# pabloconrat/our_first_climate_model

Hardware: NVIDIA B200
Metric: column*wavelength*layer flux updates/s (repwvl-100 RCE step) (higher is better)
Workload: dtype f64

## Files before the change

our_first_climate_model_b200/csrc/rcm_capi.cu:

```cuda
#include <algorithm>
#include <cmath>
#include <cstdio>
#include <cstdlib>
#include <cstring>
#include <new>
#include <functional>
#include <string>
#include <vector>

#include "rcm_diag.cuh"

#ifndef M_PI
#define M_PI 3.14159265358979323846
#endif

struct rcm_solver {
    int device = 0;
    cudaStream_t own_stream = nullptr, stream = nullptr;
    rcm_params p{};
    DevConst dc{};
    bool const_dirty = true;
    int opt_angle_cubes = 1;
    int opt_angle_pairs = 1;
    int opt_config = 0;
// ... 27 lines not shown
    bool lbl_mode = false;
    int lbl_nwvl = 0;
    double lbl_co2_factor = 1.0;
    bool lbl_has_o3_ref = false;
    double *d_lbl_lo = nullptr, *d_lbl_hi = nullptr, *d_lbl_tau5 = nullptr, *d_lbl_h2o_ref = nullptr,
           *d_lbl_o3_ref = nullptr, *d_sH = nullptr, *d_sO = nullptr, *d_dTstat = nullptr, *d_part = nullptr;
    size_t part_cap = 0;
    unsigned char* d_tile = nullptr;
    double* d_spart = nullptr;
    unsigned* d_counter = nullptr;
    unsigned* d_multi = nullptr;
    size_t multi_cap = 0;
    int opt_multi = 1;
    size_t tile_cap = 0, spart_cap = 0;
    bool tile_vmr_valid = false;
    std::vector<double> stage;
    std::string err;
    long launches = 0;
    std::vector<std::pair<cudaEvent_t, cudaEvent_t>> ev_free, ev_used;
    cudaStream_t pipe_stream[3] = {nullptr, nullptr, nullptr};
    cudaEvent_t pipe_done[3] = {nullptr, nullptr, nullptr}, pipe_start = nullptr;
    struct HostGraph {
        cudaGraphExec_t exec = nullptr;
        SplitArgs sig{};
        const void* host[7] = {};
        const void* dev[4] = {};
        double dT_converged = 0.0;
        int ncol = 0, nchunk = 0, nkernels = 0;
        long captures = 0, replays = 0;
        bool failed = false;
// ... 240 lines not shown
    CU(dalloc(s->d_rh, n * NLAY));
    CU(dalloc(s->d_Tprev, n * NLAY));
    CU(dalloc(s->d_time, n));
    CU(dalloc(s->d_Ed, n * NLEV));
    CU(dalloc(s->d_Eu, n * NLEV));
    CU(dalloc(s->d_dE, n * NLAY));
    CU(dalloc(s->d_dt, n));
    CU(dalloc(s->d_lowpos, n * NLAY));
    s->cap = ncol;
    s->diag_steps = 0;
    s->part_cap = 0;
    s->tile_cap = s->spart_cap = 0;
    s->tile_vmr_valid = false;
    if (s->d_dTstat) cudaFree(s->d_dTstat);
    s->d_dTstat = nullptr;
    if (s->d_solar_col) cudaFree(s->d_solar_col);
    if (s->d_cloud_col) cudaFree(s->d_cloud_col);
    s->d_solar_col = s->d_cloud_col = nullptr;
    s->has_col_solar = s->has_col_cloud = false;
    return RCM_OK;
}

int ensure_diag(rcm_solver* s, int nsteps) {
    if ((size_t)nsteps <= s->diag_steps && s->d_diag) return RCM_OK;
    CU(dalloc(s->d_diag, (size_t)nsteps * s->cap * 4));
    CU(dalloc(s->d_scalars, (size_t)nsteps * 4));
    CU(dalloc(s->d_red, rcm_reduce_scratch_doubles(nsteps)));
    CU(dalloc(s->d_ticket, (size_t)nsteps));
    CU(cudaMemsetAsync(s->d_ticket, 0, (size_t)nsteps * sizeof(unsigned), s->stream));
    s->diag_steps = nsteps;
// ... 90 lines not shown


bool use_split(const rcm_solver* s) {
    return !s->lbl_mode && s->has_table && s->nactive == 5 && s->opt_config == 0 && s->opt_path == 0;
}

struct SplitGeom { int ntiles, nitem, nsplit; };
SplitGeom split_geom(const rcm_solver* s, int ncols) {
    SplitGeom g;
    g.ntiles = (ncols + 15) / 16;
    g.nitem = (s->dc.nwvl + 3) / 4;
    g.nsplit = (g.nitem + rcm_split_ipu() - 1) / rcm_split_ipu();
    return g;
}

int ensure_split(rcm_solver* s) {
    const SplitGeom g = split_geom(s, s->cap);
    const size_t tiles = (size_t)g.ntiles, need_part = tiles * g.nsplit * rcm_split_part_doubles();
    if (tiles > s->tile_cap || !s->d_tile) {
        CU(dalloc(s->d_tile, tiles * rcm_split_tile_bytes()));
        s->tile_cap = tiles;
        s->tile_vmr_valid = false;
    }
    if (need_part > s->spart_cap || !s->d_spart) {
        CU(dalloc(s->d_spart, need_part));
        s->spart_cap = need_part;
    }
    if (tiles > s->multi_cap || !s->d_multi) {
        if (s->d_multi) CU(cudaFree(s->d_multi));
        s->d_multi = nullptr;
        CU(cudaMalloc((void**)&s->d_multi, 2 * tiles * sizeof(unsigned)));
        s->multi_cap = tiles;
    }
    if (!s->d_dTstat) CU(dalloc(s->d_dTstat, (size_t)s->cap));
    if (!s->d_counter) {
        CU(dalloc(s->d_counter, (size_t)4));
        CU(cudaMemsetAsync(s->d_counter, 0, 4 * sizeof(unsigned), s->stream));
    }
    return RCM_OK;
}

SplitArgs split_args(rcm_solver* s, int col0, int ncols, int which) {
    const SplitGeom g = split_geom(s, ncols);
    const size_t o = (size_t)col0, t0 = o / 16;
    SplitArgs a{};
    a.ncol = ncols;
    a.diag_ncol = s->ncol;
    a.ntiles = g.ntiles;
    a.nsplit = g.nsplit;
// ... 15 lines not shown
    a.rel_hum = s->d_rh + o * NLAY;
    a.Tprev = s->d_Tprev + o * NLAY;
    a.time_h = s->d_time + o;
    a.E_down = s->d_Ed + o * NLEV;
    a.E_up = s->d_Eu + o * NLEV;
    a.dE = s->d_dE + o * NLAY;
    a.dt = s->d_dt + o;
    a.diag = s->d_diag + o * 4;
    a.solar_col = s->has_col_solar ? s->d_solar_col + o : nullptr;
    a.cloud_col = s->has_col_cloud ? s->d_cloud_col + o : nullptr;
    a.tile = s->d_tile + t0 * rcm_split_tile_bytes();
    a.part = s->d_spart + t0 * g.nsplit * rcm_split_part_doubles();
    a.dTstat = s->d_dTstat + o;
    a.counter = s->d_counter + which;
    a.quota = 1 << 30;
    return a;
}

int split_grid(const rcm_solver* s, const SplitArgs& a, int nsm) {
    (void)s;
    if (a.quota < a.nunits) return (a.nunits + a.quota - 1) / a.quota;
    int per_sm = 3;
    if (const char* e = std::getenv("RCM_CTAS_PER_SM")) {
        const int v = std::atoi(e);
        if (v >= 1 && v < per_sm) per_sm = v;
    }
    return std::min(a.nunits, nsm * per_sm);
}

int split_rt(rcm_solver* s, const SplitArgs& a, int nsm, cudaStream_t st, bool timed) {
// ... 10 lines not shown
    }
    CU(rcm_launch_split_rt(a, split_grid(s, a, nsm), st));
    s->launches += 1;
    if (timed) {
        CU(cudaEventRecord(ev.second, st));
        s->ev_used.push_back(ev);
        if (s->ev_used.size() >= 1024) {
            const int rc = rcm_kernel_time_ms(s, 0, nullptr, nullptr);
            if (rc != RCM_OK) return rc;
        }
    }
    return RCM_OK;
}

int split_advance(rcm_solver* s, int nsteps) {
    int st = refresh_const(s);
    if (st != RCM_OK) return st;
    st = ensure_split(s);
    if (st != RCM_OK) return st;
    const int nsm = nsm_of(s);
    const SplitArgs a = split_args(s, 0, s->ncol, 0);
    SplitColFlags f{};
    f.prep = 1;
    f.first = (s->step_index == 0);
    f.write_all_vmr = !s->tile_vmr_valid;
    CU(rcm_launch_split_col(a, f, s->stream));
    s->launches += 1;
    s->tile_vmr_valid = true;
    static const int multi_rounds = std::getenv("RCM_MULTI_ROUNDS") ? std::atoi(std::getenv("RCM_MULTI_ROUNDS")) : 24;
    const int grid1 = split_grid(s, a, nsm);
    const bool few_rounds = a.nunits < (long long)multi_rounds * grid1;
    const bool fits = (long long)a.nunits * nsteps + 2LL * grid1 < (1LL << 31);
    if (nsteps >= 2 && fits && (s->opt_multi == 2 || (s->opt_multi == 1 && few_rounds))) {
        SplitMultiArgs m{};
        m.nsteps = nsteps;
        m.done = s->d_multi;
        m.ready = s->d_multi + a.ntiles;
        CU(cudaMemsetAsync(s->d_multi, 0, 2 * (size_t)a.ntiles * sizeof(unsigned), s->stream));
        SplitArgs am = a;
        am.quota = 1 << 30;
        CU(rcm_launch_split_multi(am, m, split_grid(s, am, nsm), s->stream));
        s->launches += 1;
        return RCM_OK;
    }
    for (int k = 0; k < nsteps; ++k) {
        st = split_rt(s, a, nsm, s->stream, k < 4);
        if (st != RCM_OK) return st;
        SplitColFlags e{};
        e.finish = 1;
        e.prep = (k + 1 < nsteps);
        e.first = 0;
        e.write_out = (k + 1 == nsteps);
        e.diag_step = k;
        CU(rcm_launch_split_col(a, e, s->stream));
        s->launches += 1;
    }
    return RCM_OK;
}

int launch(rcm_solver* s, int mode, int nsteps, bool want_diag) {
    int st = refresh_const(s);
    if (st != RCM_OK) return st;
    if (mode == MODE_RT ? !s->has_spectral : !s->has_table) return fail(s, RCM_ERR_STATE, "no lookup table loaded");
    if (s->ncol <= 0) return fail(s, RCM_ERR_STATE, "no columns loaded");
    const int nsm = nsm_of(s);
    Part parts[2];
    const int nparts = plan_parts(s, s->ncol, nsm, parts);
    std::pair<cudaEvent_t, cudaEvent_t> ev;
    if (!s->ev_free.empty()) {
        ev = s->ev_free.back();
        s->ev_free.pop_back();
// ... 210 lines not shown
        return RCM_ERR_CUDA;
    }
    set_active_species(s);
    *out = s;
    return RCM_OK;
}

int rcm_destroy(rcm_solver* s) {
    if (!s) return RCM_OK;
    cudaSetDevice(s->device);
    cudaStreamSynchronize(s->stream);
    if (g_const_owner[s->device & 63] == s) g_const_owner[s->device & 63] = nullptr;
    void* ptrs[] = {s->d_coef3, s->d_xsec_file, s->d_coef, s->d_species, s->d_planck_c, s->d_planck_k, s->d_exp_tab, s->d_T, s->d_Ts, s->d_vmr, s->d_rh,
                    s->d_Tprev, s->d_time, s->d_lbl_lo, s->d_lbl_hi, s->d_lbl_tau5, s->d_lbl_h2o_ref, s->d_lbl_o3_ref, s->d_sH, s->d_sO,
                    s->d_dTstat, s->d_part, s->d_Ed, s->d_Eu, s->d_dE, s->d_dt, s->d_diag, s->d_scalars, s->d_red, s->d_tau,
                    s->d_lowpos, s->d_solar_col, s->d_cloud_col, s->d_ticket, s->d_tile, s->d_spart, s->d_counter, s->d_multi, s->d_diagnose};
    for (void* q : ptrs)
        if (q) cudaFree(q);
    for (auto& e : s->ev_free) { cudaEventDestroy(e.first); cudaEventDestroy(e.second); }
    for (auto& e : s->ev_used) { cudaEventDestroy(e.first); cudaEventDestroy(e.second); }
    for (int i = 0; i < 3; ++i) {
        if (s->pipe_stream[i]) cudaStreamDestroy(s->pipe_stream[i]);
        if (s->pipe_done[i]) cudaEventDestroy(s->pipe_done[i]);
    }
    if (s->pipe_start) cudaEventDestroy(s->pipe_start);
    for (cudaStream_t q : {s->sp_up, s->sp_rt[0], s->sp_rt[1], s->sp_down})
        if (q) cudaStreamDestroy(q);
    for (int i = 0; i < 24; ++i) {
        if (s->sp_prep[i]) cudaEventDestroy(s->sp_prep[i]);
        if (s->sp_rtdone[i]) cudaEventDestroy(s->sp_rtdone[i]);
    }
// ... 1 lines not shown
    for (int i = 0; i < 2; ++i) {
        if (s->dg_stream[i]) cudaStreamDestroy(s->dg_stream[i]);
        if (s->dg_join[i]) cudaEventDestroy(s->dg_join[i]);
    }
    if (s->dg_fork) cudaEventDestroy(s->dg_fork);
    if (s->hg.exec) cudaGraphExecDestroy(s->hg.exec);
    if (s->own_stream) cudaStreamDestroy(s->own_stream);
    delete s;
    return RCM_OK;
}

const char* rcm_last_error(const rcm_solver* s) { return s ? s->err.c_str() : "null solver"; }

int rcm_set_params(rcm_solver* s, const rcm_params* p) {
    if (!s || !p) return RCM_ERR_ARG;
    if (p->nangle < 1 || p->nangle > MAX_ANGLE || p->cloud_layer >= RCM_NLAYER) return fail(s, RCM_ERR_ARG, "bad params");
    unsigned old = s->p.species_mask;
    s->p = *p;
    if (old != p->species_mask) {
        s->coef_dirty = true;
        s->ncol = 0;
    }
    s->const_dirty = true;
    set_active_species(s);
    return RCM_OK;
}

int rcm_set_option(rcm_solver* s, int option, int value) {
    if (!s) return RCM_ERR_ARG;
    if (option == 0) {
        s->opt_angle_cubes = value ? 1 : 0;
        s->const_dirty = true;
        return RCM_OK;
    }
    if (option == 1) {
        s->opt_config = value;
        s->tile_vmr_valid = false;
        return RCM_OK;
    }
    if (option == 2) {
        s->opt_cplk_narrow = value ? 1 : 0;
        return RCM_OK;
    }
    if (option == 3) {
// ... 7 lines not shown
    }
    if (option == 5) {
        s->opt_path = value ? 1 : 0;
        s->tile_vmr_valid = false;
        return RCM_OK;
    }
    if (option == 6) {
        s->opt_multi = value < 0 ? 0 : value > 2 ? 2 : value;
        return RCM_OK;
    }
    return fail(s, RCM_ERR_ARG, "unknown option");
}

int rcm_set_stream(rcm_solver* s, void* cuda_stream) {
    if (!s) return RCM_ERR_ARG;
    s->stream = cuda_stream ? (cudaStream_t)cuda_stream : s->own_stream;
    return RCM_OK;
}

int rcm_synchronize(rcm_solver* s) {
    if (!s) return RCM_ERR_ARG;
    CU(cudaSetDevice(s->device));
    CU(cudaStreamSynchronize(s->stream));
    return RCM_OK;
}

int rcm_set_repwvl_table(rcm_solver* s, const double* xsec, const double* wvl, const double* weight,
                         const double* p_grid, const double* t_ref, const double* t_pert, int n_tpert, int n_species,
                         int n_wvl, int n_p) {
    if (!s || !xsec || !wvl || !weight || !p_grid || !t_ref || !t_pert) return RCM_ERR_ARG;
    if (n_tpert < 2 || n_tpert > MAX_TPERT || n_species != RCM_NSPECIES || n_wvl < 1 || n_p < 2)
        return fail(s, RCM_ERR_ARG, "unsupported table dimensions");
    CU(cudaSetDevice(s->device));
    const size_t n = (size_t)n_tpert * n_species * n_wvl * n_p;
    CU(dalloc(s->d_xsec_file, n));
    CU(cudaMemcpy(s->d_xsec_file, xsec, n * sizeof(double), cudaMemcpyHostToDevice));
    s->coef_dirty = true;
    {
        int st = rcm_set_spectral_grid(s, wvl, weight, n_wvl);
        if (st != RCM_OK) return st;
    }
    s->p_grid.assign(p_grid, p_grid + n_p);
    s->t_ref.assign(t_ref, t_ref + n_p);
    s->t_pert.assign(t_pert, t_pert + n_tpert);
    s->dc.nwvl = n_wvl;
    s->dc.n_tpert = n_tpert;
    s->dc.n_species = n_species;
    s->dc.n_p = n_p;
    for (int m = 0; m < n_tpert; ++m) s->dc.t_pert[m] = t_pert[m];
    s->has_table = true;
    s->lbl_mode = false;
    s->const_dirty = true;
    s->tau_valid = false;
    s->tau_cap = 0;
    return RCM_OK;
}

int rcm_set_spectral_grid(rcm_solver* s, const double* wvl, const double* weight, int n_wvl) {
    if (!s || !wvl || !weight || n_wvl < 1) return RCM_ERR_ARG;
    CU(cudaSetDevice(s->device));
    const double h = 6.62607e-34, c = 299792458, kB = 1.380649e-23;
    std::vector<double> pc(n_wvl), pk(n_wvl);
    double pc_max = 0.0;
    for (int i = 0; i < n_wvl; ++i) {
        const double lam = wvl[i] * 1e-9;
        pc[i] = h * c / (lam * kB);
        pk[i] = weight[i] * 2 * h * std::pow(c, 2) / std::pow(lam, 5) / 1e9;
        if (!(wvl[i] > 0.0) || !std::isfinite(pk[i])) return fail(s, RCM_ERR_ARG, "wavelengths must be positive and finite");
        pc_max = std::max(pc_max, pc[i]);
    }
    if (pc_max / 690.0 > 20.0)
        return fail(s, RCM_ERR_ARG, "wavelengths below 1043 nm are not supported (thermal solver: the Planck exponent would leave the range of the kernels' exp)");
    s->T_floor = pc_max / 690.0;
    CU(dalloc(s->d_planck_c, (size_t)n_wvl));
// ... 11 lines not shown
    s->lbl_mode = false;
    s->const_dirty = true;
    s->tau_valid = false;
    return RCM_OK;
}

int rcm_set_repwvl_table_from(rcm_solver* s, const rcm_table* t) {
    if (!s || !t) return RCM_ERR_ARG;
    return rcm_set_repwvl_table(s, t->xsec.data(), t->wvl.data(), t->weight.data(), t->p_grid.data(), t->t_ref.data(),
                                t->t_pert.data(), t->n_tpert, t->n_species, t->n_wvl, t->n_p);
}

int rcm_set_lbl_tables(rcm_solver* s, const double* wvl, const double* tau5, int nwvl, const double* h2o_ref,
                       const double* o3_ref, double co2_factor) {
    if (!s || !wvl || !tau5 || nwvl < 2 || !h2o_ref) return RCM_ERR_ARG;
    for (int i = 1; i < nwvl; ++i)
        if (!(wvl[i] > wvl[i - 1])) return fail(s, RCM_ERR_ARG, "LBL wavelengths must be strictly ascending");
    CU(cudaSetDevice(s->device));
    std::vector<double> lo(nwvl), hi(nwvl);
    for (int i = 0; i < nwvl; ++i) {
        const double dl = (i > 0) ? (wvl[i] - wvl[i - 1]) : (wvl[1] - wvl[0]);
        const double dh = (i < nwvl - 1) ? (wvl[i + 1] - wvl[i]) : (wvl[i] - wvl[i - 1]);
        lo[i] = wvl[i] - dl / 2.0;
        hi[i] = wvl[i] + dh / 2.0;
    }
    const size_t n = (size_t)nwvl;
    CU(dalloc(s->d_lbl_lo, 4 * n));
    CU(dalloc(s->d_lbl_hi, n));
    CU(dalloc(s->d_lbl_tau5, 3 * n * NLAY));
    CU(dalloc(s->d_lbl_h2o_ref, (size_t)NLAY));
// ... 28 lines not shown
    s->lbl_mode = true;
    if (s->dc.nwvl != nwvl) {
        s->has_table = s->has_spectral = false;
        s->tau_cap = 0;
    }
    s->tau_valid = false;
    s->dc.nwvl = nwvl;
    s->const_dirty = true;
    s->part_cap = 0;
    return RCM_OK;
}

int rcm_set_columns(rcm_solver* s, int ncol, const double* plevel_hPa, const double* Tlayer, const double* Tsurf,
                    const double* vmr9, const double* rel_hum) {
    if (!s || ncol <= 0 || !plevel_hPa || !Tlayer || !Tsurf || !vmr9 || !rel_hum) return RCM_ERR_ARG;
    CU(cudaSetDevice(s->device));
    int st = ensure_columns(s, ncol);
    if (st != RCM_OK) return st;
    s->ncol = ncol;
    if (!s->has_plevel || std::memcmp(s->plevel, plevel_hPa, sizeof(s->plevel)) != 0) s->coef_dirty = true;
    std::memcpy(s->plevel, plevel_hPa, sizeof(s->plevel));
    s->has_plevel = true;
    s->const_dirty = true;
    set_active_species(s);
    const size_t n = (size_t)ncol;
    s->stage.resize(n * s->nactive * NLAY);
    for (size_t c = 0; c < n; ++c)
        for (int k = 0; k < s->nactive; ++k)
            std::memcpy(&s->stage[(c * s->nactive + k) * NLAY], vmr9 + (c * RCM_NSPECIES + s->species[k]) * NLAY,
                        NLAY * sizeof(double));
// ... 2 lines not shown
    CU(cudaMemcpyAsync(s->d_Tprev, Tlayer, n * NLAY * sizeof(double), cudaMemcpyHostToDevice, s->stream));
    CU(cudaMemcpyAsync(s->d_Ts, Tsurf, n * sizeof(double), cudaMemcpyHostToDevice, s->stream));
    CU(cudaMemcpyAsync(s->d_rh, rel_hum, n * NLAY * sizeof(double), cudaMemcpyHostToDevice, s->stream));
    CU(cudaMemsetAsync(s->d_time, 0, n * sizeof(float), s->stream));
    CU(cudaStreamSynchronize(s->stream));
    s->step_index = 0;
    s->tau_valid = false;
    s->tile_vmr_valid = false;
    s->has_col_solar = s->has_col_cloud = false;
    return RCM_OK;
}

int rcm_set_column_solar(rcm_solver* s, const rcm_solar_params* sp, const double* tau_s, const double* mu_s,
                         const double* albedo, int cloud_from_tau_s, double* solar_irr_out, double* r_total_out) {
    if (!s) return RCM_ERR_ARG;
    if (s->ncol <= 0) return fail(s, RCM_ERR_STATE, "rcm_set_columns first");
    CU(cudaSetDevice(s->device));
    if (!sp) {
        s->has_col_solar = s->has_col_cloud = false;
        s->tau_valid = false;
        return RCM_OK;
    }
    if (sp->doublings < 0 || sp->doublings > 60) return fail(s, RCM_ERR_ARG, "doublings must be in 0..60");
    if (cloud_from_tau_s && s->p.cloud_layer < 0) return fail(s, RCM_ERR_ARG, "cloud_from_tau_s needs a cloud layer");
    const size_t n = (size_t)s->ncol;
    if (!s->d_solar_col) {
        CU(dalloc(s->d_solar_col, (size_t)s->cap));
        CU(dalloc(s->d_cloud_col, (size_t)s->cap));
    }
    double* d_in = nullptr;
// ... 25 lines not shown
    if (e == cudaSuccess && r_total_out)
        e = cudaMemcpyAsync(r_total_out, d_rt, n * sizeof(double), cudaMemcpyDeviceToHost, s->stream);
    if (e == cudaSuccess) e = cudaStreamSynchronize(s->stream);
    cudaFree(d_in);
    if (d_rt) cudaFree(d_rt);
    if (e != cudaSuccess) return cuda_fail(s, e, "rcm_set_column_solar");
    s->launches += 1;
    s->has_col_solar = true;
    s->has_col_cloud = cloud_from_tau_s != 0;
    s->tau_valid = false;
    return RCM_OK;
}

int rcm_update_columns(rcm_solver* s, const double* Tlayer, const double* Tsurf, const double* vmr_active) {
    if (!s) return RCM_ERR_ARG;
    if (s->ncol <= 0) return fail(s, RCM_ERR_STATE, "rcm_set_columns first");
    CU(cudaSetDevice(s->device));
    const size_t n = (size_t)s->ncol;
    if (Tlayer) CU(cudaMemcpyAsync(s->d_T, Tlayer, n * NLAY * sizeof(double), cudaMemcpyHostToDevice, s->stream));
    if (Tsurf) CU(cudaMemcpyAsync(s->d_Ts, Tsurf, n * sizeof(double), cudaMemcpyHostToDevice, s->stream));
    if (vmr_active)
        CU(cudaMemcpyAsync(s->d_vmr, vmr_active, n * s->nactive * NLAY * sizeof(double), cudaMemcpyHostToDevice, s->stream));
    if (vmr_active) s->tile_vmr_valid = false;
    s->tau_valid = false;
    return RCM_OK;
}

int rcm_set_step_index(rcm_solver* s, long step_index) {
    if (!s || step_index < 0) return RCM_ERR_ARG;
    s->step_index = step_index;
    return RCM_OK;
}

int rcm_build_tau(rcm_solver* s, double* tau_out, int* lowpos_p, int* lowpos_t) {
    if (!s) return RCM_ERR_ARG;
    if (s->lbl_mode) return fail(s, RCM_ERR_STATE, "rcm_build_tau is the repwvl read_tau: set a repwvl table after rcm_set_lbl_tables");
    if (!s->has_table || s->ncol <= 0) return fail(s, RCM_ERR_STATE, "table and columns must be loaded");
    CU(cudaSetDevice(s->device));
    int st = ensure_tau(s);
    if (st != RCM_OK) return st;
    st = launch(s, MODE_TAU, 1, false);
    if (st != RCM_OK) return st;
    const size_t n = (size_t)s->ncol;
    if (tau_out)
        CU(cudaMemcpyAsync(tau_out, s->d_tau, n * s->dc.nwvl * NLAY * sizeof(double), cudaMemcpyDeviceToHost, s->stream));
    std::vector<int> lt;
    if (lowpos_t) CU(cudaMemcpyAsync(lowpos_t, s->d_lowpos, n * NLAY * sizeof(int), cudaMemcpyDeviceToHost, s->stream));
    CU(cudaStreamSynchronize(s->stream));
    if (lowpos_p)
        for (size_t c = 0; c < n; ++c)
            for (int k = 0; k < NLAY; ++k) lowpos_p[c * NLAY + k] = s->dc.ip[NLAY - 1 - k];
    s->tau_valid = true;
    return RCM_OK;
}

int rcm_radiative_transfer(rcm_solver* s, const double* tau, double* E_down, double* E_up, double* dE) {
    if (!s) return RCM_ERR_ARG;
    if (s->lbl_mode) return fail(s, RCM_ERR_STATE, "rcm_radiative_transfer needs a repwvl spectral grid: set one after rcm_set_lbl_tables");
    if (!s->has_spectral || s->ncol <= 0) return fail(s, RCM_ERR_STATE, "spectral grid and columns must be loaded");
    CU(cudaSetDevice(s->device));
    int st = ensure_tau(s);
    if (st != RCM_OK) return st;
    const size_t n = (size_t)s->ncol;
    if (tau) {
        CU(cudaMemcpyAsync(s->d_tau, tau, n * s->dc.nwvl * NLAY * sizeof(double), cudaMemcpyHostToDevice, s->stream));
    } else if (!s->tau_valid) {
        return fail(s, RCM_ERR_STATE, "no tau: pass one or call rcm_build_tau first");
    }
    st = launch(s, MODE_RT, 1, false);
    if (st != RCM_OK) return st;
    if (E_down) CU(cudaMemcpyAsync(E_down, s->d_Ed, n * NLEV * sizeof(double), cudaMemcpyDeviceToHost, s->stream));
    if (E_up) CU(cudaMemcpyAsync(E_up, s->d_Eu, n * NLEV * sizeof(double), cudaMemcpyDeviceToHost, s->stream));
// ... 93 lines not shown
}

int rcm_advance(rcm_solver* s, int nsteps, rcm_step_scalars* scalars_out) {
    int st = rcm_advance_async(s, nsteps, nullptr);
    if (st != RCM_OK) return st;
    if (scalars_out) {
        CU(cudaMemcpyAsync(scalars_out, s->d_scalars, (size_t)nsteps * sizeof(rcm_step_scalars), cudaMemcpyDeviceToHost,
                           s->stream));
        CU(cudaStreamSynchronize(s->stream));
    }
    return RCM_OK;
}

int rcm_run_to_equilibrium(rcm_solver* s, long max_steps, int check_every, rcm_step_scalars* last, long* steps_done) {
    if (!s || max_steps <= 0 || check_every <= 0) return RCM_ERR_ARG;
    if (steps_done) *steps_done = 0;
    std::vector<rcm_step_scalars> sc((size_t)check_every);
    long done = 0;
    while (done < max_steps) {
        const int n = (int)std::min<long>(check_every, max_steps - done);
        const int st = rcm_advance(s, n, sc.data());
        if (st != RCM_OK) return st;
        done += n;
        if (last) *last = sc[n - 1];
        if (steps_done) *steps_done = done;
        if (sc[n - 1].n_converged >= (double)s->ncol) break;
    }
    return RCM_OK;
}

// ... 11 lines not shown
    if (dE) CU(cudaMemcpyAsync(dE, s->d_dE, n * NLAY * sizeof(double), cudaMemcpyDeviceToHost, s->stream));
    if (dt) CU(cudaMemcpyAsync(dt, s->d_dt, n * sizeof(double), cudaMemcpyDeviceToHost, s->stream));
    if (h2o) {
        if (s->h2o_slot < 0) return fail(s, RCM_ERR_STATE, "H2O is not an active species");
        CU(cudaMemcpy2DAsync(h2o, NLAY * sizeof(double), s->d_vmr + (size_t)s->h2o_slot * NLAY,
                             (size_t)s->nactive * NLAY * sizeof(double), NLAY * sizeof(double), n, cudaMemcpyDeviceToHost,
                             s->stream));
    }
    CU(cudaStreamSynchronize(s->stream));
    return RCM_OK;
}

int rcm_diagnose_fluxes(rcm_solver* s, int col0, int ncol, const double* vmr_scale, double* E_down_spec, double* E_up_spec,
                        double* E_down, double* E_up, double* dE) {
    if (!s) return RCM_ERR_ARG;
    if (s->lbl_mode) return fail(s, RCM_ERR_STATE, "rcm_diagnose_fluxes: the line-by-line path is not supported");
    if (!s->has_table) return fail(s, RCM_ERR_STATE, "rcm_diagnose_fluxes: no lookup table loaded");
    if (s->ncol <= 0) return fail(s, RCM_ERR_STATE, "rcm_diagnose_fluxes: no columns loaded");
    if (s->nactive != 5) return fail(s, RCM_ERR_STATE, "rcm_diagnose_fluxes: needs the five active species of the default species_mask");
    if (!use_split(s)) return fail(s, RCM_ERR_STATE, "rcm_diagnose_fluxes: needs the split path (RCM_OPT_PATH 0, no forced tile shape)");
    if (col0 < 0 || ncol <= 0 || (long long)col0 + ncol > s->ncol)
        return fail(s, RCM_ERR_ARG, "rcm_diagnose_fluxes: columns [" + std::to_string(col0) + ", " + std::to_string((long long)col0 + ncol) +
                                        ") outside the " + std::to_string(s->ncol) + " loaded");
    DiagScale sc{};
    for (int k = 0; k < 5; ++k) {
        sc.f[k] = vmr_scale ? vmr_scale[k] : 1.0;
        if (!(sc.f[k] >= 0.0) || !std::isfinite(sc.f[k]))
            return fail(s, RCM_ERR_ARG, "rcm_diagnose_fluxes: vmr_scale[" + std::to_string(k) + "] must be finite and >= 0");
    }
    CU(cudaSetDevice(s->device));
// ... 140 lines not shown
    for (int k = 0; k < na && ok; ++k) {
        buf.resize(arr[k].bytes);
        cudaError_t e = cudaMemcpy(buf.data(), arr[k].dev, arr[k].bytes, cudaMemcpyDeviceToHost);
        if (e != cudaSuccess) {
            std::fclose(f);
            return cuda_fail(s, e, "checkpoint download");
        }
        ok = std::fwrite(buf.data(), 1, arr[k].bytes, f) == arr[k].bytes;
    }
    ok = (std::fclose(f) == 0) && ok;
    return ok ? RCM_OK : fail(s, RCM_ERR_IO, std::string("short write to ") + path);
}

int rcm_load_checkpoint(rcm_solver* s, const char* path) {
    if (!s || !path) return RCM_ERR_ARG;
    CU(cudaSetDevice(s->device));
    CU(cudaStreamSynchronize(s->stream));
    FILE* f = std::fopen(path, "rb");
    if (!f) return fail(s, RCM_ERR_IO, std::string("cannot read ") + path);
    char magic[8];
    long long hdr[8];
    double plevel[RCM_NLEVEL];
    if (std::fread(magic, 1, 8, f) != 8 || std::memcmp(magic, "RCMCKPT1", 8) != 0 || std::fread(hdr, sizeof(hdr), 1, f) != 1 ||
        std::fread(plevel, sizeof(plevel), 1, f) != 1 || hdr[0] <= 0 || hdr[0] > (1LL << 30)) {
        std::fclose(f);
        return fail(s, RCM_ERR_FORMAT, std::string(path) + " is not a checkpoint of this solver");
    }
    set_active_species(s);
    if ((unsigned)hdr[2] != s->p.species_mask || (int)hdr[1] != s->nactive) {
        std::fclose(f);
// ... 43 lines not shown
    if (!s->has_plevel || std::memcmp(s->plevel, plevel, sizeof(plevel)) != 0) s->coef_dirty = true;
    std::memcpy(s->plevel, plevel, sizeof(plevel));
    s->has_plevel = true;
    s->const_dirty = true;
    s->step_index = (long)hdr[3];
    s->has_col_solar = hdr[4] != 0;
    s->has_col_cloud = hdr[5] != 0;
    s->tau_valid = false;
    s->tile_vmr_valid = false;
    return RCM_OK;
}

int rcm_step_host(rcm_solver* s, const double* Tlayer_in, const double* Tsurf_in, const double* vmr_active_in,
                  double* E_down, double* E_up, double* dE, double* Tlayer_out, double* Tsurf_out) {
    if (!s) return RCM_ERR_ARG;
    int max_chunks = 8;
    if (const char* e = std::getenv("RCM_PIPE_CHUNKS")) max_chunks = std::max(1, std::min(16, std::atoi(e)));
    const int nchunk = (s && !s->lbl_mode && s->has_table) ? std::min(max_chunks, s->ncol / 4096) : 0;
    if (nchunk < 2) {
        int st = rcm_update_columns(s, Tlayer_in, Tsurf_in, vmr_active_in);
        if (st != RCM_OK) return st;
        st = rcm_advance_async(s, 1, nullptr);
        if (st != RCM_OK) return st;
        return rcm_get_state(s, Tlayer_out, Tsurf_out, nullptr, nullptr, E_down, E_up, dE, nullptr);
    }
    CU(cudaSetDevice(s->device));
    int st = ensure_diag(s, 1);
    if (st != RCM_OK) return st;
    st = refresh_const(s);
    if (st != RCM_OK) return st;
// ... 130 lines not shown
```

our_first_climate_model_b200/csrc/rcm_kernels.cuh:

```cuda
#ifndef RCM_KERNELS_CUH
#define RCM_KERNELS_CUH

#include <cuda_runtime.h>

#include "rcm_internal.h"

constexpr int NLAY = RCM_NLAYER;
constexpr int NLEV = RCM_NLEVEL;
constexpr int MAX_ANGLE = 64;
constexpr int MAX_TPERT = 16;
constexpr int PLK_MAX = 128;
constexpr int MAX_PAIR = 16;
constexpr int HALF = NLAY / 2;
constexpr int RCM_LBL_C = 16, RCM_LBL_NT = 128;
#ifndef RCM_EXP_LOG2
#define RCM_EXP_LOG2 10
#endif
constexpr int EXP_LOG2 = RCM_EXP_LOG2, EXP_TAB = 1 << EXP_LOG2;
constexpr int EXP_REP = (EXP_LOG2 == 7) ? 8 : 1;
#ifdef RCM_EXP_DEG_OVERRIDE
constexpr int EXP_DEG = RCM_EXP_DEG_OVERRIDE;
#else
constexpr int EXP_DEG = (EXP_LOG2 == 7) ? 3 : 2;
#endif
// ... 84 lines not shown
    int ntiles, nsplit, ipu, nitem, nunits;
    int stage_rows, clampk, h2o_slot;
    double tau_clamp, T_floor;
    const double* __restrict__ coef;
    const double* __restrict__ planck_c;
    const double* __restrict__ planck_k;
    const double* __restrict__ exp_tab;
    double* Tlayer; double* Tsurf; double* vmr; const double* rel_hum; double* Tprev; float* time_h;
    double* E_down; double* E_up; double* dE; double* dt; double* diag;
    const double* solar_col; const double* cloud_col;
    unsigned char* tile;
    double* part;
    double* dTstat;
    unsigned* counter;
    int quota;
};
struct SplitColFlags {
    int finish;
    int prep;
    int first;
    int write_all_vmr;
    int write_out;
    int diag_step;
};
struct SplitMultiArgs {
    int nsteps;
    unsigned* done;
    unsigned* ready;
};
size_t rcm_split_tile_bytes();
size_t rcm_split_part_doubles();
int rcm_split_ipu();
cudaError_t rcm_launch_split_col(const SplitArgs& a, const SplitColFlags& f, cudaStream_t st);
cudaError_t rcm_launch_split_rt(const SplitArgs& a, int grid, cudaStream_t st);
cudaError_t rcm_launch_split_multi(const SplitArgs& a, const SplitMultiArgs& m, int grid, cudaStream_t st);

enum { MODE_STEP = 0, MODE_TAU = 1, MODE_RT = 2 };

// ... 25 lines not shown
```

our_first_climate_model_b200/csrc/rcm_split_kernels.cuh:

```cuda
#pragma once

constexpr int SPLIT_C = 16, SPLIT_NT = 128, SPLIT_G = 4;
constexpr int SPLIT_IPU = 5;
constexpr int SPLIT_COL_NT = 128;

constexpr int TB_INVT = 0;
constexpr int TB_DELT = TB_INVT + TBD_LEN;
constexpr int TB_DTDP = TB_DELT + TBD_LEN;
constexpr int TB_VMR = TB_DTDP + TBD_LEN;
constexpr int TB_INVTS = TB_VMR + 5 * TBD_LEN;
constexpr int TB_CLOUD = TB_INVTS + SPLIT_C;
constexpr int TB_DOUBLES = TB_CLOUD + SPLIT_C;
constexpr int TBI_IT = 0;
constexpr int TBI_ROWSEL = TBI_IT + TBI_LEN;
constexpr int TBI_ROWOFF = TBI_ROWSEL + TBI_LEN;
constexpr int TBI_OUTSIDE = TBI_ROWOFF + NLAY * NCAND;
constexpr int TB_INTS = (TBI_OUTSIDE + 1 + 3) / 4 * 4;
constexpr int TILE_BYTES = TB_DOUBLES * 8 + TB_INTS * 4;
static_assert(TILE_BYTES % 16 == 0, "bulk copies move multiples of 16 bytes");
constexpr int ROWB3 = 16 * 8;
constexpr int ROWS3 = ROWB3 + 16;
constexpr int ROWBUF3 = NLAY * NCAND * ROWS3;
constexpr int SPLIT_PART = 2 * NLEV * SPLIT_C;

// ... 9 lines not shown
    double* const sT = cs.sT; double* const sTh = cs.sTh; double* const sPrev = cs.sPrev; double* const sRh = cs.sRh;
    double* const sEd = cs.sEd; double* const sEu = cs.sEu; double* const sdE = cs.sdE; double* const sdt = cs.sdt;
    double* const sTs = cs.sTs; double* const sSol = cs.sSol; double* const sStat = cs.sStat;
    int* const sit = cs.sit; int* const sitmin = cs.sitmin; int* const sout = cs.sout;
    int extrap = 0;
    const int tid = threadIdx.x;
    const int col0 = tile * C, ncl = min(C, a.ncol - col0);
    const int nact = cst.nactive, nwvl = cst.nwvl;
    if (STANDALONE && tile == 0 && tid == 0 && a.counter) *a.counter = 0u;
    double* const tb = reinterpret_cast<double*>(a.tile + (size_t)tile * TILE_BYTES);
    int* const tbi = reinterpret_cast<int*>(tb + TB_DOUBLES);
    const bool feedback = f.prep && !f.first && a.h2o_slot >= 0;
    for (int i = tid; i < LC; i += NT) {
        const int cc = i / NLAY, l = i % NLAY;
        const size_t gi = (size_t)(col0 + (cc < ncl ? cc : 0)) * NLAY + l;
        sT[l * C + cc] = __ldcg(a.Tlayer + gi);
        if (f.prep) sPrev[l * C + cc] = __ldcg(a.Tprev + gi);
        if (feedback) sRh[l * C + cc] = a.rel_hum[gi];
    }
    if (tid < C) {
        const int col = col0 + (tid < ncl ? tid : 0);
        sTs[tid] = __ldcg(a.Tsurf + col);
        sSol[tid] = a.solar_col ? a.solar_col[col] : cst.solar_irr;
        if (f.finish) sStat[tid] = __ldcg(a.dTstat + col);
    }
    if (f.finish) {
        const double* part = a.part + (size_t)tile * a.nsplit * SPLIT_PART;
        for (int i = tid; i < SPLIT_PART; i += NT) {
            const int row = i / C;
            double sum = 0.0;
            if (row != NLAY)
                for (int sp = 0; sp < a.nsplit; ++sp) sum += __ldcg(part + (size_t)sp * SPLIT_PART + i);
            if (row < NLAY) sEd[i + C] = sum;
            else if (row == NLAY) sEd[i % C] = 0.0;
            else sEu[i - NLEV * C] = sum;
        }
    }
    __syncthreads();

// ... 37 lines not shown
            if (l == NLAY - 1) {
                const double ts = Tn * cst.conv[NLAY - 1];
                sTs[cc] = ts;
                if (cc < ncl) a.Tsurf[col0 + cc] = ts;
            }
        }
        if (f.write_out) {
            for (int i = tid; i < NLEV * ncl; i += NT) {
                const int cc = i / NLEV, l = i % NLEV;
                a.E_down[(size_t)col0 * NLEV + i] = sEd[l * C + cc];
                a.E_up[(size_t)col0 * NLEV + i] = sEu[l * C + cc];
            }
            for (int i = tid; i < NLAY * ncl; i += NT) a.dE[(size_t)col0 * NLAY + i] = sdE[(i % NLAY) * C + i / NLAY];
        }
        __syncthreads();
        if (!f.prep) {
            for (int i = tid; i < NLAY * ncl; i += NT) a.Tlayer[(size_t)col0 * NLAY + i] = sT[(i % NLAY) * C + i / NLAY];
            return;
        }
    }

    auto indices = [&] {
        for (int i = tid; i < LC; i += NT) {
            const int l = i / C, cc = i % C, r = prow(l);
            const double midT = sT[i], tref = cst.tref_ip[r];
            const int it = lowerpos_t(tref, midT, cst.n_tpert);
            const double t0 = tref + cst.t_pert[it], t1 = tref + cst.t_pert[it + 1];
            extrap |= (midT < tref + cst.t_pert[0]) | (midT > tref + cst.t_pert[cst.n_tpert - 1]);
            sit[r * C + cc] = it;
            tbi[TBI_IT + tbix(r, cc)] = it;
            const double dT = (midT - t0) / (t1 - t0);
            tb[TB_DELT + tbd(r, cc)] = dT;
            tb[TB_DTDP + tbd(r, cc)] = __dmul_rn(dT, cst.delP[r]);
        }
// ... 5 lines not shown
        const int l = i / C, cc = i % C;
        const double my = sTh[i];
        int rank = 0;
#pragma unroll
        for (int l2 = 0; l2 < NLAY; ++l2) {
            const double v = sTh[l2 * C + cc];
            rank += (v > my || (v == my && l2 < l)) ? 1 : 0;
        }
        const double Tn = my / cst.conv[rank];
        sT[rank * C + cc] = Tn;
        sdE[rank * C + cc] = fabs(Tn - sPrev[rank * C + cc]);
    }
    __syncthreads();
    for (int i = tid; i < NLAY * ncl; i += NT) {
        const double v = sT[(i % NLAY) * C + i / NLAY];
        a.Tlayer[(size_t)col0 * NLAY + i] = v;
        a.Tprev[(size_t)col0 * NLAY + i] = v;
    }
    if (tid < ncl) {
        double dmax = 0.0;
#pragma unroll
        for (int l = 0; l < NLAY; ++l) dmax = fmax(dmax, sdE[l * C + tid]);
        a.dTstat[col0 + tid] = dmax;
    }
    for (int i = tid; i < nact * LC; i += NT) {
        const int cc = i % C, l = (i / C) % NLAY, sp = i / LC;
        const bool h2o = (sp == a.h2o_slot) && !f.first;
        if (!h2o && !f.write_all_vmr) continue;
        double v = 0.0;
        if (cc < ncl) {
            const size_t gi = ((size_t)(col0 + cc) * nact + sp) * NLAY + l;
            if (h2o) {
                const double Tc = sT[l * C + cc] - 273.15;
                const double e_sat = 6.1094 * exp(17.625 * Tc / (Tc + 243.04));
                v = sRh[l * C + cc] * e_sat / cst.player[l];
                a.vmr[gi] = v;
            } else {
                v = a.vmr[gi];
            }
        }
        tb[TB_VMR + sp * TBD_LEN + tbd(prow(l), cc)] = v;
    }
    if (!f.first) indices();
    for (int i = tid; i < LC; i += NT) tb[TB_INVT + tbd(prow(i / C), i % C)] = (1.0 / fmax(sT[i], a.T_floor)) * L2E64;
    if (tid < C) {
        tb[TB_INVTS + tid] = (1.0 / fmax(sTs[tid], a.T_floor)) * L2E64;
        tb[TB_CLOUD + tid] = a.cloud_col ? a.cloud_col[col0 + (tid < ncl ? tid : 0)] : cst.cloud_tau;
    }
    const int any_extrap = __syncthreads_or(extrap);
    if (tid < NLAY) {
        int mn = sit[tid * C], mx = mn;
// ... 90 lines not shown
```

Measured before the change: 40.17 billion.

## Prepare next step's tile inputs ahead in final finish kernel via shadow buffers

The last finish launch of a split_advance call now also runs the prep stage for the following call. It writes the adjusted temperatures, dTstat and water-vapour vmr into shadow buffers so the visible state stays unchanged. On the next call, if nothing invalidated the prepared state, the separate prep launch is skipped and the first finish kernel copies the shadow values back. This removes one kernel launch and a full column read per call, at the cost of extra shadow buffers, more state to keep valid, and extra prep work whenever the prepared result gets thrown away.

```diff
diff --git a/our_first_climate_model_b200/csrc/rcm_capi.cu b/our_first_climate_model_b200/csrc/rcm_capi.cu
--- a/our_first_climate_model_b200/csrc/rcm_capi.cu
+++ b/our_first_climate_model_b200/csrc/rcm_capi.cu
@@ -65,6 +65,8 @@
     int opt_multi = 1;
     size_t tile_cap = 0, spart_cap = 0;
     bool tile_vmr_valid = false;
+    bool prepared = false;
+    double *d_Tsh = nullptr, *d_dTstatsh = nullptr, *d_h2osh = nullptr;
     std::vector<double> stage;
     std::string err;
     long launches = 0;
@@ -335,6 +337,11 @@
     s->tile_vmr_valid = false;
     if (s->d_dTstat) cudaFree(s->d_dTstat);
     s->d_dTstat = nullptr;
+    for (double** p : {&s->d_Tsh, &s->d_dTstatsh, &s->d_h2osh}) {
+        if (*p) cudaFree(*p);
+        *p = nullptr;
+    }
+    s->prepared = false;
     if (s->d_solar_col) cudaFree(s->d_solar_col);
     if (s->d_cloud_col) cudaFree(s->d_cloud_col);
     s->d_solar_col = s->d_cloud_col = nullptr;
@@ -455,6 +462,8 @@
     return g;
 }
 
+void drop_prepared(rcm_solver* s) { s->prepared = false; }
+
 int ensure_split(rcm_solver* s) {
     const SplitGeom g = split_geom(s, s->cap);
     const size_t tiles = (size_t)g.ntiles, need_part = tiles * g.nsplit * rcm_split_part_doubles();
@@ -474,6 +483,11 @@
         s->multi_cap = tiles;
     }
     if (!s->d_dTstat) CU(dalloc(s->d_dTstat, (size_t)s->cap));
+    if (!s->d_Tsh) {
+        CU(dalloc(s->d_Tsh, (size_t)s->cap * NLAY));
+        CU(dalloc(s->d_dTstatsh, (size_t)s->cap));
+        CU(dalloc(s->d_h2osh, (size_t)s->cap * NLAY));
+    }
     if (!s->d_counter) {
         CU(dalloc(s->d_counter, (size_t)4));
         CU(cudaMemsetAsync(s->d_counter, 0, 4 * sizeof(unsigned), s->stream));
@@ -519,6 +533,9 @@
     a.dTstat = s->d_dTstat + o;
     a.counter = s->d_counter + which;
     a.quota = 1 << 30;
+    a.Tsh = s->d_Tsh ? s->d_Tsh + o * NLAY : nullptr;
+    a.dTstatsh = s->d_dTstatsh ? s->d_dTstatsh + o : nullptr;
+    a.h2osh = s->d_h2osh ? s->d_h2osh + o * NLAY : nullptr;
     return a;
 }
 
@@ -559,24 +576,30 @@
 }
 
 int split_advance(rcm_solver* s, int nsteps) {
+    const bool prepared = s->prepared;
+    s->prepared = false;
     int st = refresh_const(s);
     if (st != RCM_OK) return st;
     st = ensure_split(s);
     if (st != RCM_OK) return st;
     const int nsm = nsm_of(s);
     const SplitArgs a = split_args(s, 0, s->ncol, 0);
-    SplitColFlags f{};
-    f.prep = 1;
-    f.first = (s->step_index == 0);
-    f.write_all_vmr = !s->tile_vmr_valid;
-    CU(rcm_launch_split_col(a, f, s->stream));
-    s->launches += 1;
-    s->tile_vmr_valid = true;
     static const int multi_rounds = std::getenv("RCM_MULTI_ROUNDS") ? std::atoi(std::getenv("RCM_MULTI_ROUNDS")) : 24;
     const int grid1 = split_grid(s, a, nsm);
     const bool few_rounds = a.nunits < (long long)multi_rounds * grid1;
     const bool fits = (long long)a.nunits * nsteps + 2LL * grid1 < (1LL << 31);
-    if (nsteps >= 2 && fits && (s->opt_multi == 2 || (s->opt_multi == 1 && few_rounds))) {
+    const bool multi = nsteps >= 2 && fits && (s->opt_multi == 2 || (s->opt_multi == 1 && few_rounds));
+    const bool from_shadow = prepared && !multi;
+    if (!from_shadow) {
+        SplitColFlags f{};
+        f.prep = 1;
+        f.first = (s->step_index == 0);
+        f.write_all_vmr = !s->tile_vmr_valid;
+        CU(rcm_launch_split_col(a, f, s->stream));
+        s->launches += 1;
+        s->tile_vmr_valid = true;
+    }
+    if (multi) {
         SplitMultiArgs m{};
         m.nsteps = nsteps;
         m.done = s->d_multi;
@@ -588,18 +611,22 @@
         s->launches += 1;
         return RCM_OK;
     }
+    const bool ahead = s->opt_multi != 0;
     for (int k = 0; k < nsteps; ++k) {
         st = split_rt(s, a, nsm, s->stream, k < 4);
         if (st != RCM_OK) return st;
         SplitColFlags e{};
         e.finish = 1;
-        e.prep = (k + 1 < nsteps);
+        e.prep = (k + 1 < nsteps) || ahead;
         e.first = 0;
         e.write_out = (k + 1 == nsteps);
         e.diag_step = k;
+        e.from_shadow = (k == 0 && from_shadow);
+        e.to_shadow = ahead && (k + 1 == nsteps);
         CU(rcm_launch_split_col(a, e, s->stream));
         s->launches += 1;
     }
+    s->prepared = ahead;
     return RCM_OK;
 }
 
@@ -840,7 +867,8 @@
     void* ptrs[] = {s->d_coef3, s->d_xsec_file, s->d_coef, s->d_species, s->d_planck_c, s->d_planck_k, s->d_exp_tab, s->d_T, s->d_Ts, s->d_vmr, s->d_rh,
                     s->d_Tprev, s->d_time, s->d_lbl_lo, s->d_lbl_hi, s->d_lbl_tau5, s->d_lbl_h2o_ref, s->d_lbl_o3_ref, s->d_sH, s->d_sO,
                     s->d_dTstat, s->d_part, s->d_Ed, s->d_Eu, s->d_dE, s->d_dt, s->d_diag, s->d_scalars, s->d_red, s->d_tau,
-                    s->d_lowpos, s->d_solar_col, s->d_cloud_col, s->d_ticket, s->d_tile, s->d_spart, s->d_counter, s->d_multi, s->d_diagnose};
+                    s->d_lowpos, s->d_solar_col, s->d_cloud_col, s->d_ticket, s->d_tile, s->d_spart, s->d_counter, s->d_multi, s->d_diagnose,
+                    s->d_Tsh, s->d_dTstatsh, s->d_h2osh};
     for (void* q : ptrs)
         if (q) cudaFree(q);
     for (auto& e : s->ev_free) { cudaEventDestroy(e.first); cudaEventDestroy(e.second); }
@@ -872,6 +900,7 @@
 
 int rcm_set_params(rcm_solver* s, const rcm_params* p) {
     if (!s || !p) return RCM_ERR_ARG;
+    drop_prepared(s);
     if (p->nangle < 1 || p->nangle > MAX_ANGLE || p->cloud_layer >= RCM_NLAYER) return fail(s, RCM_ERR_ARG, "bad params");
     unsigned old = s->p.species_mask;
     s->p = *p;
@@ -886,6 +915,7 @@
 
 int rcm_set_option(rcm_solver* s, int option, int value) {
     if (!s) return RCM_ERR_ARG;
+    drop_prepared(s);
     if (option == 0) {
         s->opt_angle_cubes = value ? 1 : 0;
         s->const_dirty = true;
@@ -923,6 +953,7 @@
 
 int rcm_set_stream(rcm_solver* s, void* cuda_stream) {
     if (!s) return RCM_ERR_ARG;
+    drop_prepared(s);
     s->stream = cuda_stream ? (cudaStream_t)cuda_stream : s->own_stream;
     return RCM_OK;
 }
@@ -938,6 +969,7 @@
                          const double* p_grid, const double* t_ref, const double* t_pert, int n_tpert, int n_species,
                          int n_wvl, int n_p) {
     if (!s || !xsec || !wvl || !weight || !p_grid || !t_ref || !t_pert) return RCM_ERR_ARG;
+    drop_prepared(s);
     if (n_tpert < 2 || n_tpert > MAX_TPERT || n_species != RCM_NSPECIES || n_wvl < 1 || n_p < 2)
         return fail(s, RCM_ERR_ARG, "unsupported table dimensions");
     CU(cudaSetDevice(s->device));
@@ -967,6 +999,7 @@
 
 int rcm_set_spectral_grid(rcm_solver* s, const double* wvl, const double* weight, int n_wvl) {
     if (!s || !wvl || !weight || n_wvl < 1) return RCM_ERR_ARG;
+    drop_prepared(s);
     CU(cudaSetDevice(s->device));
     const double h = 6.62607e-34, c = 299792458, kB = 1.380649e-23;
     std::vector<double> pc(n_wvl), pk(n_wvl);
@@ -1008,6 +1041,7 @@
 int rcm_set_lbl_tables(rcm_solver* s, const double* wvl, const double* tau5, int nwvl, const double* h2o_ref,
                        const double* o3_ref, double co2_factor) {
     if (!s || !wvl || !tau5 || nwvl < 2 || !h2o_ref) return RCM_ERR_ARG;
+    drop_prepared(s);
     for (int i = 1; i < nwvl; ++i)
         if (!(wvl[i] > wvl[i - 1])) return fail(s, RCM_ERR_ARG, "LBL wavelengths must be strictly ascending");
     CU(cudaSetDevice(s->device));
@@ -1066,6 +1100,7 @@
 int rcm_set_columns(rcm_solver* s, int ncol, const double* plevel_hPa, const double* Tlayer, const double* Tsurf,
                     const double* vmr9, const double* rel_hum) {
     if (!s || ncol <= 0 || !plevel_hPa || !Tlayer || !Tsurf || !vmr9 || !rel_hum) return RCM_ERR_ARG;
+    drop_prepared(s);
     CU(cudaSetDevice(s->device));
     int st = ensure_columns(s, ncol);
     if (st != RCM_OK) return st;
@@ -1098,6 +1133,7 @@
 int rcm_set_column_solar(rcm_solver* s, const rcm_solar_params* sp, const double* tau_s, const double* mu_s,
                          const double* albedo, int cloud_from_tau_s, double* solar_irr_out, double* r_total_out) {
     if (!s) return RCM_ERR_ARG;
+    drop_prepared(s);
     if (s->ncol <= 0) return fail(s, RCM_ERR_STATE, "rcm_set_columns first");
     CU(cudaSetDevice(s->device));
     if (!sp) {
@@ -1153,6 +1189,7 @@
 
 int rcm_update_columns(rcm_solver* s, const double* Tlayer, const double* Tsurf, const double* vmr_active) {
     if (!s) return RCM_ERR_ARG;
+    drop_prepared(s);
     if (s->ncol <= 0) return fail(s, RCM_ERR_STATE, "rcm_set_columns first");
     CU(cudaSetDevice(s->device));
     const size_t n = (size_t)s->ncol;
@@ -1167,12 +1204,14 @@
 
 int rcm_set_step_index(rcm_solver* s, long step_index) {
     if (!s || step_index < 0) return RCM_ERR_ARG;
+    drop_prepared(s);
     s->step_index = step_index;
     return RCM_OK;
 }
 
 int rcm_build_tau(rcm_solver* s, double* tau_out, int* lowpos_p, int* lowpos_t) {
     if (!s) return RCM_ERR_ARG;
+    drop_prepared(s);
     if (s->lbl_mode) return fail(s, RCM_ERR_STATE, "rcm_build_tau is the repwvl read_tau: set a repwvl table after rcm_set_lbl_tables");
     if (!s->has_table || s->ncol <= 0) return fail(s, RCM_ERR_STATE, "table and columns must be loaded");
     CU(cudaSetDevice(s->device));
@@ -1195,6 +1234,7 @@
 
 int rcm_radiative_transfer(rcm_solver* s, const double* tau, double* E_down, double* E_up, double* dE) {
     if (!s) return RCM_ERR_ARG;
+    drop_prepared(s);
     if (s->lbl_mode) return fail(s, RCM_ERR_STATE, "rcm_radiative_transfer needs a repwvl spectral grid: set one after rcm_set_lbl_tables");
     if (!s->has_spectral || s->ncol <= 0) return fail(s, RCM_ERR_STATE, "spectral grid and columns must be loaded");
     CU(cudaSetDevice(s->device));
@@ -1318,6 +1358,7 @@
 
 int rcm_run_to_equilibrium(rcm_solver* s, long max_steps, int check_every, rcm_step_scalars* last, long* steps_done) {
     if (!s || max_steps <= 0 || check_every <= 0) return RCM_ERR_ARG;
+    drop_prepared(s);
     if (steps_done) *steps_done = 0;
     std::vector<rcm_step_scalars> sc((size_t)check_every);
     long done = 0;
@@ -1359,6 +1400,7 @@
 int rcm_diagnose_fluxes(rcm_solver* s, int col0, int ncol, const double* vmr_scale, double* E_down_spec, double* E_up_spec,
                         double* E_down, double* E_up, double* dE) {
     if (!s) return RCM_ERR_ARG;
+    drop_prepared(s);
     if (s->lbl_mode) return fail(s, RCM_ERR_STATE, "rcm_diagnose_fluxes: the line-by-line path is not supported");
     if (!s->has_table) return fail(s, RCM_ERR_STATE, "rcm_diagnose_fluxes: no lookup table loaded");
     if (s->ncol <= 0) return fail(s, RCM_ERR_STATE, "rcm_diagnose_fluxes: no columns loaded");
@@ -1529,6 +1571,7 @@
 
 int rcm_load_checkpoint(rcm_solver* s, const char* path) {
     if (!s || !path) return RCM_ERR_ARG;
+    drop_prepared(s);
     CU(cudaSetDevice(s->device));
     CU(cudaStreamSynchronize(s->stream));
     FILE* f = std::fopen(path, "rb");
@@ -1602,6 +1645,7 @@
 int rcm_step_host(rcm_solver* s, const double* Tlayer_in, const double* Tsurf_in, const double* vmr_active_in,
                   double* E_down, double* E_up, double* dE, double* Tlayer_out, double* Tsurf_out) {
     if (!s) return RCM_ERR_ARG;
+    drop_prepared(s);
     int max_chunks = 8;
     if (const char* e = std::getenv("RCM_PIPE_CHUNKS")) max_chunks = std::max(1, std::min(16, std::atoi(e)));
     const int nchunk = (s && !s->lbl_mode && s->has_table) ? std::min(max_chunks, s->ncol / 4096) : 0;
diff --git a/our_first_climate_model_b200/csrc/rcm_kernels.cuh b/our_first_climate_model_b200/csrc/rcm_kernels.cuh
--- a/our_first_climate_model_b200/csrc/rcm_kernels.cuh
+++ b/our_first_climate_model_b200/csrc/rcm_kernels.cuh
@@ -122,6 +122,7 @@
     double* dTstat;
     unsigned* counter;
     int quota;
+    double* Tsh; double* dTstatsh; double* h2osh;
 };
 struct SplitColFlags {
     int finish;
@@ -130,6 +131,7 @@
     int write_all_vmr;
     int write_out;
     int diag_step;
+    int from_shadow = 0, to_shadow = 0;
 };
 struct SplitMultiArgs {
     int nsteps;
diff --git a/our_first_climate_model_b200/csrc/rcm_split_kernels.cuh b/our_first_climate_model_b200/csrc/rcm_split_kernels.cuh
--- a/our_first_climate_model_b200/csrc/rcm_split_kernels.cuh
+++ b/our_first_climate_model_b200/csrc/rcm_split_kernels.cuh
@@ -47,15 +47,26 @@
     for (int i = tid; i < LC; i += NT) {
         const int cc = i / NLAY, l = i % NLAY;
         const size_t gi = (size_t)(col0 + (cc < ncl ? cc : 0)) * NLAY + l;
-        sT[l * C + cc] = __ldcg(a.Tlayer + gi);
-        if (f.prep) sPrev[l * C + cc] = __ldcg(a.Tprev + gi);
+        if (f.from_shadow) {
+            const double t = __ldcg(a.Tsh + gi);
+            sT[l * C + cc] = t;
+            sPrev[l * C + cc] = t;
+            if (cc < ncl) {
+                a.Tprev[gi] = t;
+                if (a.h2o_slot >= 0) a.vmr[((size_t)(col0 + cc) * nact + a.h2o_slot) * NLAY + l] = __ldcg(a.h2osh + gi);
+            }
+        } else {
+            sT[l * C + cc] = __ldcg(a.Tlayer + gi);
+            if (f.prep) sPrev[l * C + cc] = __ldcg(a.Tprev + gi);
+        }
         if (feedback) sRh[l * C + cc] = a.rel_hum[gi];
     }
     if (tid < C) {
         const int col = col0 + (tid < ncl ? tid : 0);
         sTs[tid] = __ldcg(a.Tsurf + col);
         sSol[tid] = a.solar_col ? a.solar_col[col] : cst.solar_irr;
-        if (f.finish) sStat[tid] = __ldcg(a.dTstat + col);
+        if (f.finish) sStat[tid] = __ldcg((f.from_shadow ? a.dTstatsh : a.dTstat) + col);
+        if (f.from_shadow && tid < ncl) a.dTstat[col] = sStat[tid];
     }
     if (f.finish) {
         const double* part = a.part + (size_t)tile * a.nsplit * SPLIT_PART;
@@ -123,10 +134,9 @@
             for (int i = tid; i < NLAY * ncl; i += NT) a.dE[(size_t)col0 * NLAY + i] = sdE[(i % NLAY) * C + i / NLAY];
         }
         __syncthreads();
-        if (!f.prep) {
+        if (!f.prep || f.to_shadow)
             for (int i = tid; i < NLAY * ncl; i += NT) a.Tlayer[(size_t)col0 * NLAY + i] = sT[(i % NLAY) * C + i / NLAY];
-            return;
-        }
+        if (!f.prep) return;
     }
 
     auto indices = [&] {
@@ -162,14 +172,18 @@
     __syncthreads();
     for (int i = tid; i < NLAY * ncl; i += NT) {
         const double v = sT[(i % NLAY) * C + i / NLAY];
-        a.Tlayer[(size_t)col0 * NLAY + i] = v;
-        a.Tprev[(size_t)col0 * NLAY + i] = v;
+        if (f.to_shadow) {
+            a.Tsh[(size_t)col0 * NLAY + i] = v;
+        } else {
+            a.Tlayer[(size_t)col0 * NLAY + i] = v;
+            a.Tprev[(size_t)col0 * NLAY + i] = v;
+        }
     }
     if (tid < ncl) {
         double dmax = 0.0;
 #pragma unroll
         for (int l = 0; l < NLAY; ++l) dmax = fmax(dmax, sdE[l * C + tid]);
-        a.dTstat[col0 + tid] = dmax;
+        (f.to_shadow ? a.dTstatsh : a.dTstat)[col0 + tid] = dmax;
     }
     for (int i = tid; i < nact * LC; i += NT) {
         const int cc = i % C, l = (i / C) % NLAY, sp = i / LC;
@@ -182,7 +196,8 @@
                 const double Tc = sT[l * C + cc] - 273.15;
                 const double e_sat = 6.1094 * exp(17.625 * Tc / (Tc + 243.04));
                 v = sRh[l * C + cc] * e_sat / cst.player[l];
-                a.vmr[gi] = v;
+                if (f.to_shadow) a.h2osh[(size_t)(col0 + cc) * NLAY + l] = v;
+                else a.vmr[gi] = v;
             } else {
                 v = a.vmr[gi];
             }
```

Result: no change. 40.19 billion (median of 6 runs) (+0.0%).
